# IONIQ6000/av1-go

Hardware: AMD Instinct MI355X
Metric: encoded 4K30 frames/sec (whole node) at fixed QP; PSNR-Y delta vs libaom (higher is better)
Workload: dtype u16

## Files before the change

### av1-go_amd/csrc/av1_entropy_kernels.hip

```cpp
#include <string.h>
#include <vector>
#include "av1_ops_cdfs.hpp"
#include "av1_ops32.hpp"
#include "av1mi_internal.hpp"

namespace av1mi {
using namespace av1ops;

struct Av1EntLaunch {
  FrameView fv;
  int nframes, sbr_n, sbc_n;
  BlockInfo *info;
  op_t *ops; uint32_t ops_cap;
  uint32_t *grouped; uint32_t grouped_cap;
  uint16_t *slot_total, *slot_base;
  uint16_t *rec;
  uint32_t *nops;
  uint8_t *slots; uint32_t slot_cap;
  uint32_t *tile_size;
  uint64_t *tile_off;
  uint32_t *status;
  uint8_t *out; uint64_t out_cap;
  const uint16_t *cdf_image; int cdf_words;
  SlotTable tab;
  const uint16_t *cdf_image32; SlotTable tab32;
  const uint8_t *lr_on_frame;
  int sb_rows32, band, nslots;
};

__device__ __forceinline__ FrameView frame_view(const Av1EntLaunch &L, int f) {
  FrameView v = L.fv;
  const long nb = (long)v.w8 * v.h8;
  if (v.key) { v.y_mode += nb * f; v.uv_mode += nb * f; }
  else { v.mv += nb * 2 * f; v.skip += nb * f; }
  v.lev_y += nb * 64 * f; v.lev_u += nb * 16 * f; v.lev_v += nb * 16 * f;
  v.info = L.info + nb * f;
  if (L.lr_on_frame) for (int p = 0; p < 3; p++) v.lr_on[p] = v.lr_on[p] && L.lr_on_frame[f * 3 + p];
  return v;
}

__global__ __launch_bounds__(256) void k_av1_info(Av1EntLaunch L) {
  const long nb = (long)L.fv.w8 * L.fv.h8, i = (long)blockIdx.x * 256 + threadIdx.x;
  if (i >= nb * L.nframes) return;
  const int f = (int)(i / nb), b = (int)(i - (long)f * nb);
  const FrameView v = frame_view(L, f);
  BlockInfo o = {};
  block_summary(v, b, &o);
  if (!v.key) inter_mode_decision(v, b / v.w8, b % v.w8, &o);
  L.info[nb * f + b] = o;
}

constexpr int kReplaySlots = (S_MAX + 1) / 2;
// ... 70 lines not shown
    if (sl >= S_MAX) continue;
    const bool on = sl < nslots;
    L.slot_total[(size_t)t * S_MAX + sl] = on ? S.total[sl] : (uint16_t)0;
    L.slot_base[(size_t)t * S_MAX + sl] = on ? S.base[sl] : (uint16_t)0;
  }
  op_t *list = L.ops + (size_t)t * L.ops_cap;
  uint32_t *grouped = L.grouped + (size_t)t * L.grouped_cap;
#pragma unroll
  for (int half = 0; half < 2; half++) {
    const int lo = half * kReplaySlots, hi = lo + kReplaySlots;
    if (half) __syncthreads();
#pragma unroll
    for (int q = 0; q < kOwn; q++) {
      const int sl = zi + 64 * q;
      if (sl < lo || sl >= hi || sl >= nslots) continue;
      int run = S.base[sl];
#pragma unroll
      for (int w = 0; w < kBlocksPerTile / 4; w++) {
        const uint32_t u = c[q][w];
        const int p0 = run, p1 = p0 + (int)(u & 0xFF), p2 = p1 + (int)((u >> 8) & 0xFF), p3 = p2 + (int)((u >> 16) & 0xFF);
        run = p3 + (int)(u >> 24);
        uint32_t *d = reinterpret_cast<uint32_t *>(S.pos + (sl - lo) * kBlocksPerTile + 4 * w);
        d[0] = (uint32_t)p0 | ((uint32_t)p1 << 16); d[1] = (uint32_t)p2 | ((uint32_t)p3 << 16);
      }
    }
    __syncthreads();
    __threadfence_block();
    replay_block(rec, k.nrec, S.pos, zi, first, list, grouped, lo, hi, half == 0);
  }
}

constexpr int kTiles32 = 16;
static_assert(kBlocks32 * kMag32Bytes >= K_END * kBlocks32 * 2 && kMag32Bytes % 8 == 0, "a tile's counters live where its four magnitude maps were");
__global__ __launch_bounds__(64) void k_av1_tokens32(Av1EntLaunch L, int ntiles_all) {
  __shared__ ScanTables32 scan;
  __shared__ __attribute__((aligned(16))) uint8_t s_mag[64 * kMag32Bytes];
  __shared__ Sum32 s_sum[kTiles32][kBlocks32];
  __shared__ int s_n[kTiles32][kBlocks32], s_nrec[kTiles32][kBlocks32], s_bad[kTiles32];
  const int tiles = L.sbr_n * L.sbc_n, tl = threadIdx.x >> 2, b = threadIdx.x & 3, t = blockIdx.x * kTiles32 + tl;
  bool live = t < ntiles_all;
  int f = 0, sbr = 0, sbc = 0;
  if (live) { f = t / tiles; const int tt = t - f * tiles; sbr = tt / L.sbc_n; sbc = tt - sbr * L.sbc_n; live = sbr < L.sb_rows32; }
  fill_scan_tables32(&scan, (int)threadIdx.x, 64);
  if (b == 0) s_bad[tl] = 0;
  const FrameView v = frame_view(L, live ? f : 0);
  const bool inside = live && !((b & 1) && sbc * 8 + 4 >= v.w8);
  if (inside) block_sums32(v, block_index32(v, sbr, sbc, b), &s_sum[tl][b]);
  __syncthreads();
  uint16_t *rec = L.rec + ((size_t)(live ? t : 0) * kBlocks32 + b) * kBlockRecords32;
  int nrec = 0;
  if (live) { s_n[tl][b] = 0; s_nrec[tl][b] = 0; }
  if (inside) {
    Sink32 k = { rec, nullptr, b, (int)kBlockRecords32, 0, 0, false, 0, 0, 0, 0 };
    const TokScratch32 ts = { s_mag + threadIdx.x * kMag32Bytes, &scan };
    tok_block32(v, k, ts, sbr, sbc, b, s_sum[tl]);
    s_n[tl][b] = k.n; s_nrec[tl][b] = nrec = k.nrec;
    if (k.overflow) atomicOr(&s_bad[tl], 1);
  }
  __syncthreads();
  uint16_t *cnt = reinterpret_cast<uint16_t *>(s_mag + tl * kBlocks32 * kMag32Bytes);
  for (int i = b; i < K_END * kBlocks32; i += kBlocks32) cnt[i] = 0;
  __syncthreads();
  if (live && !count_block32(rec, nrec, cnt, b)) atomicOr(&s_bad[tl], 1);
  __syncthreads();
  if (live && b == 0) {
    uint16_t *total = L.slot_total + (size_t)t * S_MAX, *base = L.slot_base + (size_t)t * S_MAX;
    const int run = place_tile32(cnt, total, base);
    for (int sl = K_END; sl < S_MAX; sl++) { total[sl] = 0; base[sl] = 0; }
    const int n = s_n[tl][0] + s_n[tl][1] + s_n[tl][2] + s_n[tl][3];
    if (s_bad[tl] || (uint32_t)n > L.ops_cap || run > 65535) {
      s_bad[tl] = 1;
      atomicOr(L.status, 1u);
      L.nops[t] = 0;
      for (int sl = 0; sl < K_END; sl++) total[sl] = 0;
    } else {
      L.nops[t] = (uint32_t)n;
    }
  }
  __syncthreads();
  if (!live || s_bad[tl]) return;
  int first = 0;
  for (int q = 0; q < b; q++) first += s_n[tl][q];
  replay_block32(rec, nrec, cnt, b, first, L.ops + (size_t)t * L.ops_cap, L.grouped + (size_t)t * L.grouped_cap);
}

__global__ __launch_bounds__(64) void k_av1_chains(Av1EntLaunch L, int ntiles_all, int ngroups) {
  const int xcd = blockIdx.x & 7, j = blockIdx.x >> 3, nslots = L.nslots;
  const int g = (j / nslots) * 8 + xcd, sl = j - (j / nslots) * nslots, lane = threadIdx.x, t = g * 64 + lane;
  if (g >= ngroups) return;
// ... 13 lines not shown
    const uint4 *g4 = reinterpret_cast<const uint4 *>(grouped);
    const uint4 z = make_uint4(0, 0, 0, 0);
    uint4 c0 = cnt > 0 ? g4[0] : z, c1 = cnt > 4 ? g4[1] : z, c2 = cnt > 8 ? g4[2] : z, c3 = cnt > 12 ? g4[3] : z;
    auto four = [&](const uint4 &v, int e) {
      if (e < cnt) list[v.x >> 4] = small_step(cdf, (int)(v.x & 15), n);
      if (e + 1 < cnt) list[v.y >> 4] = small_step(cdf, (int)(v.y & 15), n);
      if (e + 2 < cnt) list[v.z >> 4] = small_step(cdf, (int)(v.z & 15), n);
      if (e + 3 < cnt) list[v.w >> 4] = small_step(cdf, (int)(v.w & 15), n);
    };
#pragma unroll 1
    for (int e = 0; e < cnt; e += 16) {
      const uint4 *nx = g4 + (e >> 2) + 4;
      const uint4 n0 = e + 16 < cnt ? nx[0] : z, n1 = e + 20 < cnt ? nx[1] : z, n2 = e + 24 < cnt ? nx[2] : z, n3 = e + 28 < cnt ? nx[3] : z;
      four(c0, e); four(c1, e + 4); four(c2, e + 8); four(c3, e + 12);
      c0 = n0; c1 = n1; c2 = n2; c3 = n3;
    }
  } else {
    uint16_t *cdf = s_big + lane * 16;
    {
      const uint4 *iw = reinterpret_cast<const uint4 *>(L.cdf_image + off);
      uint4 *d = reinterpret_cast<uint4 *>(cdf);
      d[0] = iw[0];
      d[1] = n > 8 ? iw[1] : make_uint4(0, 0, 0, 0);
    }
#pragma unroll 1
    for (int e = 0; e < cnt; e++) {
      const uint32_t v = grouped[e];
      const int s = (int)(v & 15);
      list[v >> 4] = s >= kSplitHorz ? split_tuple(cdf, s) : big_step(cdf, s, n);
    }
  }
}

constexpr int kRingOps = 64, kLaneWords = kRingOps * 2 + Coder::kStage + 8;

__global__ __launch_bounds__(64) void k_av1_code(Av1EntLaunch L, int ntiles_all) {
  __shared__ __attribute__((aligned(16))) uint16_t s_lane[64 * kLaneWords];
  const int lane = threadIdx.x, t = blockIdx.x * 64 + lane;
  const bool live = t < ntiles_all;
  uint32_t *ring = reinterpret_cast<uint32_t *>(s_lane + lane * kLaneWords);
  Coder c;
  c.init(L.slots + (size_t)(live ? t : 0) * L.slot_cap, (int)L.slot_cap, s_lane + lane * kLaneWords + kRingOps * 2);
  const int n = live ? (int)L.nops[t] : 0;
  const uint4 *ops4 = reinterpret_cast<const uint4 *>(L.ops + (size_t)(live ? t : 0) * L.ops_cap);
  uint4 r0, r1, r2, r3, r4, r5, r6, r7;
  r0 = r1 = r2 = r3 = r4 = r5 = r6 = r7 = make_uint4(0, 0, 0, 0);
  int w = 0;
  bool pend = false;
  auto request = [&]() {
    const uint4 *p = ops4 + (w >> 2);
    if (w < n) r0 = p[0];
    if (w + 4 < n) r1 = p[1];
    if (w + 8 < n) r2 = p[2];
    if (w + 12 < n) r3 = p[3];
    if (w + 16 < n) r4 = p[4];
    if (w + 20 < n) r5 = p[5];
    if (w + 24 < n) r6 = p[6];
    if (w + 28 < n) r7 = p[7];
    pend = w < n;
  };
  auto take = [&]() {
    uint4 *q = reinterpret_cast<uint4 *>(ring + (w & 32));
    q[0] = r0; q[1] = r1; q[2] = r2; q[3] = r3; q[4] = r4; q[5] = r5; q[6] = r6; q[7] = r7;
    w += 32;
  };
  request();
  if (pend) { take(); request(); }
  int i = 0, lit_left = 0;
  uint32_t op = ring[0], op_next = ring[1], op_next2 = ring[2];
  for (;;) {
    if (!__any(lit_left > 0 || i < n)) break;
    if (__any((pend && w - i < 24) || c.ns >= Coder::kStage - 8)) {
      if (pend && w - i <= 32) { take(); request(); }
      c.spill();
    }
#pragma unroll
    for (int q = 0; q < 8; q++) {
      if (lit_left > 0 || i < n) {
        const uint32_t fetched = ring[(i + 3) & (kRingOps - 1)];
        uint32_t tup = op;
        if (lit_left == 0 && (op >> 31)) lit_left = (int)((op >> 27) & 15);
        if (lit_left > 0) {
          lit_left--;
          tup = (op >> lit_left) & 1 ? (1u << 19) | (256u << 9) : (2u << 19) | (512u << 9) | 256u;
        }
        c.encode_tuple(tup);
        if (lit_left == 0) { i++; op = op_next; op_next = op_next2; op_next2 = fetched; }
      }
    }
  }
  if (!live) return;
  int sz = n ? c.finish() : -1;
  if (sz < 0) { if (n) atomicOr(L.status, 2u); sz = 0; }
  L.tile_size[t] = (uint32_t)sz;
}

__global__ __launch_bounds__(1024) void k_av1_scan(Av1EntLaunch L, int ntiles_all) {
  __shared__ uint64_t part[1024];
  const int tid = threadIdx.x, per = (ntiles_all + 1023) / 1024, i0 = tid * per, i1 = min(i0 + per, ntiles_all);
  uint64_t s = 0;
  for (int i = i0; i < i1; i++) s += L.tile_size[i];
  part[tid] = s;
  __syncthreads();
  for (int d = 1; d < 1024; d <<= 1) {
    const uint64_t y = tid >= d ? part[tid - d] : 0;
    __syncthreads();
    part[tid] += y;
    __syncthreads();
  }
  uint64_t run = part[tid] - s;
  for (int i = i0; i < i1; i++) { L.tile_off[i] = run; run += L.tile_size[i]; }
  if (tid == 1023) {
    L.tile_off[ntiles_all] = part[1023];
    if (part[1023] > L.out_cap) atomicOr(L.status, 4u);
  }
}
__global__ __launch_bounds__(64) void k_av1_gather(Av1EntLaunch L) {
  const int t = blockIdx.x;
  const uint32_t n = L.tile_size[t];
  const uint64_t off = L.tile_off[t];
  if (off + n > L.out_cap) return;
  const uint8_t *src = L.slots + (size_t)t * L.slot_cap;
  uint8_t *dst = L.out + off;
  const uint32_t head = min(n, (uint32_t)((16 - (reinterpret_cast<uintptr_t>(dst) & 15)) & 15)), body = (n - head) >> 4, tail0 = head + (body << 4);
  if (threadIdx.x < head) dst[threadIdx.x] = src[threadIdx.x];
  for (uint32_t i = threadIdx.x; i < body; i += 64) {
    uint4 v;
    __builtin_memcpy(&v, src + head + 16 * i, 16);
    *reinterpret_cast<uint4 *>(dst + head + 16 * i) = v;
  }
  if (tail0 + threadIdx.x < n) dst[tail0 + threadIdx.x] = src[tail0 + threadIdx.x];
}

hipError_t launch_av1_front(av1mi_ctx *ctx, const Av1EntLaunch &L, hipStream_t s) {
  const long nb = (long)L.fv.w8 * L.fv.h8 * L.nframes;
  const int ntiles_all = L.sbr_n * L.sbc_n * L.nframes, ngroups = (ntiles_all + 63) / 64;
  ProfToken t = ctx_prof_begin(ctx, AV1MI_K_ENTROPY_TOKENS, s);
  hipLaunchKernelGGL(k_av1_info, dim3((unsigned)((nb + 255) / 256)), dim3(256), 0, s, L);
  if (L.sb_rows32 < L.sbr_n) hipLaunchKernelGGL(k_av1_tokens, dim3((unsigned)ntiles_all), dim3(64), 0, s, L);
  if (L.sb_rows32) hipLaunchKernelGGL(k_av1_tokens32, dim3((unsigned)((ntiles_all + kTiles32 - 1) / kTiles32)), dim3(64), 0, s, L, ntiles_all);
  ctx_prof_end(ctx, t, s);
  t = ctx_prof_begin(ctx, AV1MI_K_ENTROPY_CHAINS, s);
  Av1EntLaunch C = L;
  C.nslots = L.fv.key ? S_KEY_END : S_INTER_END; C.band = L.sb_rows32 ? 2 : 0;
  if (L.sb_rows32 < L.sbr_n) hipLaunchKernelGGL(k_av1_chains, dim3((unsigned)(((ngroups + 7) / 8) * 8 * C.nslots)), dim3(64), 0, s, C, ntiles_all, ngroups);
  if (L.sb_rows32) {
    C.nslots = K_END; C.band = 1; C.tab = L.tab32; C.cdf_image = L.cdf_image32;
    hipLaunchKernelGGL(k_av1_chains, dim3((unsigned)(((ngroups + 7) / 8) * 8 * C.nslots)), dim3(64), 0, s, C, ntiles_all, ngroups);
  }
  ctx_prof_end(ctx, t, s);
  return hipGetLastError();
}
hipError_t launch_av1_back(av1mi_ctx *ctx, const Av1EntLaunch &L, hipStream_t s) {
  const int ntiles_all = L.sbr_n * L.sbc_n * L.nframes;
  ProfToken t = ctx_prof_begin(ctx, AV1MI_K_ENTROPY, s);
  hipLaunchKernelGGL(k_av1_code, dim3((unsigned)((ntiles_all + 63) / 64)), dim3(64), 0, s, L, ntiles_all);
  ctx_prof_end(ctx, t, s);
  t = ctx_prof_begin(ctx, AV1MI_K_ENTROPY_PACK, s);
  hipLaunchKernelGGL(k_av1_scan, dim3(1), dim3(1024), 0, s, L, ntiles_all);
  hipLaunchKernelGGL(k_av1_gather, dim3((unsigned)ntiles_all), dim3(64), 0, s, L);
  ctx_prof_end(ctx, t, s);
  return hipGetLastError();
}

}

struct av1mi_av1ent_state {
  void *info = nullptr, *ops[2] = { nullptr, nullptr }, *nops[2] = { nullptr, nullptr }, *grouped = nullptr, *slot_tb = nullptr, *rec = nullptr, *slots = nullptr, *tile_off = nullptr, *status = nullptr;
  size_t info_b = 0, ops_b[2] = { 0, 0 }, nops_b[2] = { 0, 0 }, grouped_b = 0, slot_tb_b = 0, rec_b = 0, slots_b = 0, off_b = 0;
  hipEvent_t lists_ready[2] = { nullptr, nullptr }, lists_free[2] = { nullptr, nullptr };
  bool free_recorded[2] = { false, false };
  unsigned long jobs = 0;
  av1mi::Av1EntLaunch pending[2];
  uint64_t *pending_total[2] = { nullptr, nullptr };
  bool pending_valid[2] = { false, false };
  size_t last_tiles = 0;
  uint16_t *d_image[2][4] = {};
  uint16_t *d_image32[4] = {};
  av1ops::SlotTable tab32;
  int image_words[2] = { 0, 0 };
  av1ops::SlotTable tab[2];
};

namespace {
int grow(av1mi_ctx *ctx, void **p, size_t *have, size_t need) {
  if (*have >= need) return AV1MI_OK;
  if (*p) (void)hipFree(*p);
  *p = nullptr; *have = 0;
  if (hipMalloc(p, need) != hipSuccess) return av1mi::ctx_fail(ctx, AV1MI_E_NOMEM, "AV1 entropy scratch: hipMalloc(%zu) failed", need);
  *have = need;
  return AV1MI_OK;
}
}

extern "C" {

uint32_t av1mi_av1_entropy_ops_per_tile(void) { return 32768; }
uint32_t av1mi_av1_entropy_slot_bytes(void) { return 16384; }

}

int av1mi::av1_entropy_front(av1mi_ctx *ctx, const av1mi_av1_entropy_job *j, hipStream_t front, int *ticket) {
// ... 23 lines not shown
    return av1mi::ctx_fail(ctx, AV1MI_E_INVAL, "key_rows32 %d: whole superblock rows of a key frame whose width is a multiple of 32", j->key_rows32);
  if (j->key_rows32 && !st->d_image32[qcat]) {
    const std::vector<uint16_t> img = av1ops::default_slot_image_k32(qcat, &st->tab32);
    if (hipMalloc((void **)&st->d_image32[qcat], img.size() * 2) != hipSuccess ||
        hipMemcpy(st->d_image32[qcat], img.data(), img.size() * 2, hipMemcpyHostToDevice) != hipSuccess)
      return av1mi::ctx_fail(ctx, AV1MI_E_DEVICE, "uploading the default CDF image failed");
  }
  av1mi::Av1EntLaunch L;
  memset(&L, 0, sizeof(L));
  L.sb_rows32 = j->key_rows32 / 64;
  if (j->key_rows32) { av1ops::build_slot_table_k32(&L.tab32); L.cdf_image32 = st->d_image32[qcat]; }
  L.fv.w8 = j->width / 8; L.fv.h8 = j->height / 8; L.fv.key = key;
  L.fv.y_mode = j->d_modes_y; L.fv.uv_mode = j->d_modes_uv; L.fv.mv = j->d_mvs; L.fv.skip = j->d_skip;
  L.fv.lev_y = j->d_lev_y; L.fv.lev_u = j->d_lev_u; L.fv.lev_v = j->d_lev_v;
  for (int p = 0; p < 3; p++) {
    L.fv.lr_on[p] = j->lr_on[p] != 0;
    const int vh = j->visible_height ? j->visible_height : j->height, vw = j->visible_width ? j->visible_width : j->width;
    const int ph = p ? (vh + 1) / 2 : vh, pw = p ? (vw + 1) / 2 : vw;
    L.fv.lr_rows[p] = (ph + 32) / 64 > 1 ? (ph + 32) / 64 : 1; L.fv.lr_cols[p] = (pw + 32) / 64 > 1 ? (pw + 32) / 64 : 1;
  }
  memcpy(L.fv.lr_unit[0], j->lr_unit_y, 8); memcpy(L.fv.lr_unit[1], j->lr_unit_uv, 8);
  L.nframes = j->nframes; L.sbr_n = (L.fv.h8 + 7) / 8; L.sbc_n = (L.fv.w8 + 7) / 8;
  const size_t nb = (size_t)L.fv.w8 * L.fv.h8 * j->nframes, nt = (size_t)L.sbr_n * L.sbc_n * j->nframes;
  L.ops_cap = av1mi_av1_entropy_ops_per_tile(); L.slot_cap = av1mi_av1_entropy_slot_bytes();
  L.grouped_cap = L.ops_cap + av1ops::kListAlign * av1ops::S_MAX;
  const int par = (int)(st->jobs++ & 1);
  st->last_tiles = nt;
  int rc;
  if ((rc = grow(ctx, &st->info, &st->info_b, nb * sizeof(av1ops::BlockInfo))) ||
      (rc = grow(ctx, &st->ops[par], &st->ops_b[par], nt * L.ops_cap * sizeof(av1ops::op_t))) || (rc = grow(ctx, &st->nops[par], &st->nops_b[par], nt * 4)) ||
      (rc = grow(ctx, &st->grouped, &st->grouped_b, nt * L.grouped_cap * sizeof(uint32_t))) ||
      (rc = grow(ctx, &st->slot_tb, &st->slot_tb_b, nt * av1ops::S_MAX * 4)) ||
      (rc = grow(ctx, &st->rec, &st->rec_b, nt * av1ops::kBlocksPerTile * av1ops::kBlockRecords * sizeof(uint16_t))) ||
      (rc = grow(ctx, &st->slots, &st->slots_b, nt * L.slot_cap)) || (rc = grow(ctx, &st->tile_off, &st->off_b, (nt + 1) * 8)))
    return rc;
  L.info = (av1ops::BlockInfo *)st->info; L.ops = (av1ops::op_t *)st->ops[par]; L.nops = (uint32_t *)st->nops[par]; L.grouped = (uint32_t *)st->grouped;
  L.slot_total = (uint16_t *)st->slot_tb; L.slot_base = L.slot_total + nt * av1ops::S_MAX; L.rec = (uint16_t *)st->rec; L.slots = (uint8_t *)st->slots;
  L.tile_off = (uint64_t *)st->tile_off;
  L.tile_size = j->d_tile_size; L.out = j->d_out; L.out_cap = j->out_cap;
  L.status = (uint32_t *)(j->d_total + 1);
  L.cdf_image = st->d_image[key][qcat]; L.cdf_words = st->image_words[key]; L.tab = st->tab[key];
  L.lr_on_frame = j->d_lr_on;
#define E_HIP(call) do { const hipError_t e_ = (call); if (e_ != hipSuccess) return av1mi::ctx_fail(ctx, AV1MI_E_DEVICE, "%s: %s", #call, hipGetErrorString(e_)); } while (0)
  for (hipEvent_t *ev : { &st->lists_ready[par], &st->lists_free[par] }) if (!*ev) E_HIP(hipEventCreateWithFlags(ev, hipEventDisableTiming));
  if (st->free_recorded[par]) E_HIP(hipStreamWaitEvent(front, st->lists_free[par], 0));
  E_HIP(hipMemsetAsync(j->d_total, 0, 16, front));
  E_HIP(av1mi::launch_av1_front(ctx, L, front));
  E_HIP(hipEventRecord(st->lists_ready[par], front));
  st->pending[par] = L; st->pending_total[par] = j->d_total; st->pending_valid[par] = true;
  *ticket = par;
  return AV1MI_OK;
}

int av1mi::av1_entropy_back(av1mi_ctx *ctx, int ticket, hipStream_t back) {
  if (!ctx || ticket < 0 || ticket > 1) return AV1MI_E_INVAL;
  av1mi_av1ent_state *st = av1mi::ctx_av1ent(ctx);
  if (!st || !st->pending_valid[ticket]) return av1mi::ctx_fail(ctx, AV1MI_E_INVAL, "no entropy job pending under this ticket");
  const av1mi::Av1EntLaunch &L = st->pending[ticket];
  const size_t nt = (size_t)L.sbr_n * L.sbc_n * L.nframes;
  E_HIP(hipStreamWaitEvent(back, st->lists_ready[ticket], 0));
  E_HIP(av1mi::launch_av1_back(ctx, L, back));
  E_HIP(hipMemcpyAsync(st->pending_total[ticket], L.tile_off + nt, 8, hipMemcpyDeviceToDevice, back));
  E_HIP(hipEventRecord(st->lists_free[ticket], back)); st->free_recorded[ticket] = true;
  st->pending_valid[ticket] = false;
#undef E_HIP
  return AV1MI_OK;
}

int av1mi::av1_entropy_submit(av1mi_ctx *ctx, const av1mi_av1_entropy_job *j, hipStream_t front, hipStream_t back) {
  int ticket = -1;
  const int rc = av1_entropy_front(ctx, j, front, &ticket);
  if (rc != AV1MI_OK || ticket < 0) return rc;
  return av1_entropy_back(ctx, ticket, back);
}

extern "C" {

int av1mi_av1_entropy_encode_on(av1mi_ctx *ctx, const av1mi_av1_entropy_job *j, void *stream_handle) {
  if (!ctx) return AV1MI_E_INVAL;
  hipStream_t s = stream_handle ? (hipStream_t)stream_handle : av1mi::ctx_stream(ctx);
  return av1mi::av1_entropy_submit(ctx, j, s, s);
}

int av1mi_av1_entropy_encode(av1mi_ctx *ctx, const av1mi_av1_entropy_job *j) { return av1mi_av1_entropy_encode_on(ctx, j, nullptr); }

int av1mi_av1_entropy_last_list_words(av1mi_ctx *ctx, uint64_t *words) {
  if (!ctx || !words) return AV1MI_E_INVAL;
  *words = 0;
  av1mi_av1ent_state *st = av1mi::ctx_av1ent(ctx);
  if (!st || !st->jobs || !st->last_tiles) return AV1MI_OK;
  if (hipSetDevice(av1mi::ctx_device(ctx)) != hipSuccess || hipDeviceSynchronize() != hipSuccess) return av1mi::ctx_fail(ctx, AV1MI_E_DEVICE, "synchronising failed");
  std::vector<uint32_t> n(st->last_tiles);
  if (hipMemcpy(n.data(), st->nops[(st->jobs - 1) & 1], n.size() * 4, hipMemcpyDeviceToHost) != hipSuccess) return av1mi::ctx_fail(ctx, AV1MI_E_DEVICE, "reading the list sizes failed");
  for (uint32_t v : n) *words += v;
  return AV1MI_OK;
}

}

namespace av1mi {
void av1ent_free(av1mi_av1ent_state *st) {
  if (!st) return;
  for (void *p : { st->info, st->ops[0], st->ops[1], st->nops[0], st->nops[1], st->grouped, st->slot_tb, st->rec, st->slots, st->tile_off }) if (p) (void)hipFree(p);
  for (hipEvent_t ev : { st->lists_ready[0], st->lists_ready[1], st->lists_free[0], st->lists_free[1] }) if (ev) (void)hipEventDestroy(ev);
  for (auto &k : st->d_image) for (uint16_t *p : k) if (p) (void)hipFree(p);
  delete st;
}
av1mi_av1ent_state *av1ent_new() { return new (std::nothrow) av1mi_av1ent_state(); }
}
```

### av1-go_amd/csrc/av1_ops.hpp

```cpp
#pragma once
#include <stdint.h>

#if defined(__HIPCC__)
#include <hip/hip_runtime.h>
#define AV1_HD __host__ __device__ inline
#define AV1_UNROLL _Pragma("unroll")
#define AV1_NOUNROLL _Pragma("unroll 1")
#else
#define AV1_HD inline
#define AV1_UNROLL
#define AV1_NOUNROLL
#endif

namespace av1ops {

typedef uint32_t __attribute__((may_alias)) u32a;
typedef uint64_t __attribute__((may_alias)) u64a;

enum Slot : int {
  S_SKIP = 0,
  S_PART8 = S_SKIP + 3,
  S_PART16 = S_PART8 + 1,
  S_PART32 = S_PART16 + 4,
  S_PART64 = S_PART32 + 4,
// ... 591 lines not shown
    if (k >= nd) continue;
    uint32_t lo = adapt(w[k] & 0xFFFFu, 2 * k < s, rate), hi = adapt(w[k] >> 16, 2 * k + 1 < s, rate);
    if (k == nd - 1) hi = cnt + (cnt < 32);
    d[k] = lo | (hi << 16);
  }
  return make_tuple(fl, fh, s, n);
}

AV1_HD op_t split_tuple(const uint16_t *p, int kind) {
  const uint32_t p1 = p[0] - p[1], p2 = p[1] - p[2], p3 = p[2] - p[3], p4 = p[3] - p[4], p5 = p[4] - p[5], p6 = p[5] - p[6], p7 = p[6] - p[7],
                 p8 = p[7] - p[8], p9 = p[8];
  return make_tuple(kind == kSplitHorz ? p2 + p3 + p4 + p6 + p7 + p9 : p1 + p3 + p4 + p5 + p6 + p8, 0, 1, 2);
}

AV1_HD void run_chain(const uint16_t *init, int n, const uint32_t *g, int cnt, op_t *list) {
  if (n <= 4) {
    uint64_t w = (uint64_t)init[0] | ((uint64_t)init[1] << 16) | ((uint64_t)init[2] << 32) | ((uint64_t)init[3] << 48);
    for (int k = 0; k < cnt; k++) list[g[k] >> 4] = small_step(w, (int)(g[k] & 15), n);
    return;
  }
  alignas(16) uint16_t v[16];
  for (int i = 0; i < 16; i++) v[i] = i < slot_words(n) ? init[i] : 0;
  for (int k = 0; k < cnt; k++) {
    const int s = (int)(g[k] & 15);
    list[g[k] >> 4] = s >= kSplitHorz ? split_tuple(v, s) : big_step(v, s, n);
  }
}

AV1_HD void code_word(Coder &c, op_t e) {
  if (e >> 31) { for (int i = (int)((e >> 27) & 15) - 1; i >= 0; i--) { c.bit((e >> i) & 1); if (c.stage_full()) c.spill(); } }
  else { c.encode_tuple(e); if (c.stage_full()) c.spill(); }
}

}
```

### av1-go_amd/host/av1_opstream.cpp

```cpp
#include <algorithm>
#include <cstdio>
#include <cstdlib>
#include <cstring>
#include <string>
#include <vector>
#include "../csrc/av1_ops_cdfs.hpp"
#include "av1_bitstream.hpp"

namespace av1mi_host {
namespace av1 {

bool opstream_supported(const av1mi_obu_frame &f, std::string *why) {
  auto no = [&](const char *m) { if (why) *why = m; return false; };
  if (f.cdef_bits || f.reduced_tx_set || f.disable_cdf_update) return no("cdef_bits / reduced_tx_set / disable_cdf_update must be 0");
  if (f.tile_cols_log2 >= 0 || f.tile_rows_log2 >= 0) return no("one superblock per tile only");
  if (f.angle_y || f.angle_uv || f.cfl_alpha || f.tx_type || f.is_inter) return no("angle deltas, chroma from luma, transform types and intra blocks in inter frames are host-writer only");
  if (f.frame_type == 0 && f.skip) return no("key frames are coded with skip = 0");
  for (int p = 0; p < 3; p++) if (f.lr_type[p] > 1) return no("Wiener restoration only");
  if (f.lr_unit_shift || f.lr_uv_shift) return no("64x64 restoration units only");
  return true;
}

bool opstream_tiles(const av1mi_obu_frame &f, std::vector<std::vector<uint8_t>> *tiles, std::string *err, int key_rows32) {
  using namespace av1ops;
  if (!opstream_supported(f, err)) return false;
  if (key_rows32 && (f.frame_type != 0 || (key_rows32 & 63) || key_rows32 > f.height || (f.width & 31))) { if (err) *err = "bad 32x32 band"; return false; }
  FrameView v;
  memset(&v, 0, sizeof(v));
  v.w8 = f.width / 8; v.h8 = f.height / 8; v.key = f.frame_type == 0;
  v.y_mode = f.y_mode; v.uv_mode = f.uv_mode; v.mv = f.mv; v.skip = f.skip; v.lev_y = f.lev_y; v.lev_u = f.lev_u; v.lev_v = f.lev_v;
  std::vector<uint8_t> zskip;
  if (!v.key && !v.skip) { zskip.assign((size_t)v.w8 * v.h8, 0); v.skip = zskip.data(); }
  for (int p = 0; p < 3; p++) {
    v.lr_on[p] = f.lr_type[p] == 1;
    const int ph = p ? (visible_height(f) + 1) >> 1 : visible_height(f), pw = p ? (visible_width(f) + 1) >> 1 : visible_width(f);
    v.lr_rows[p] = std::max((ph + 32) / 64, 1); v.lr_cols[p] = std::max((pw + 32) / 64, 1);
  }
  for (int p = 0; p < 3; p++) {
    if (!v.lr_on[p]) continue;
    const int8_t *u = f.lr_units[p];
    const size_t n = (size_t)v.lr_rows[p] * v.lr_cols[p];
    for (size_t i = 1; i < n; i++) if (memcmp(u, u + i * 8, 8)) { if (err) *err = "restoration units must be uniform per plane"; return false; }
    if (p == 2 && v.lr_on[1] && memcmp(u, f.lr_units[1], 8)) { if (err) *err = "U and V restoration units must be equal"; return false; }
    memcpy(v.lr_unit[p ? 1 : 0], u, 8);
  }
  const size_t nb = (size_t)v.w8 * v.h8;
  std::vector<BlockInfo> info(nb);
  v.info = info.data();
  for (size_t b = 0; b < nb; b++) { memset(&info[b], 0, sizeof(BlockInfo)); block_summary(v, (int)b, &info[b]); }
  if (!v.key) for (int r = 0; r < v.h8; r++) for (int c = 0; c < v.w8; c++) inter_mode_decision(v, r, c, &info[(size_t)r * v.w8 + c]);
  const int qcat = f.base_q_idx <= 20 ? 0 : f.base_q_idx <= 60 ? 1 : f.base_q_idx <= 120 ? 2 : 3;
  SlotTable tab;
  const std::vector<uint16_t> image = default_slot_image(v.key != 0, qcat, &tab);
// ... 21 lines not shown
      if (sbr * 64 < key_rows32) {
        std::fill(cnt32.begin(), cnt32.end(), 0);
        const TokScratch32 ts32 = { mag32, scan32.data() };
        Sum32 sums[kBlocks32];
        const bool half = sbc * 8 + 4 >= v.w8;
        for (int b = 0; b < kBlocks32; b++) if (!(half && (b & 1))) block_sums32(v, block_index32(v, sbr, sbc, b), &sums[b]);
        int nrec[kBlocks32], first[kBlocks32 + 1];
        first[0] = 0;
        for (int b = 0; b < kBlocks32; b++) {
          Sink32 k = { &rec32[(size_t)b * kBlockRecords32], cnt32.data(), b, (int)kBlockRecords32, 0, 0, false, 0, 0, 0, 0 };
          tok_block32(v, k, ts32, sbr, sbc, b, sums);
          if (k.overflow) { if (err) *err = "a block exceeds the tokenizer's record area"; return false; }
          nrec[b] = k.nrec; first[b + 1] = first[b] + k.n;
        }
        for (int b = 0; b < kBlocks32; b++)
          if (!count_block32(&rec32[(size_t)b * kBlockRecords32], nrec[b], cnt32.data(), b)) { if (err) *err = "too many symbols of one slot in a block"; return false; }
        uint16_t base[K_END], total[K_END];
        const int run = place_tile32(cnt32.data(), total, base);
        if (run > 65535) { if (err) *err = "tile too large for 16-bit entry positions"; return false; }
        const int nops = first[kBlocks32];
        list.assign((size_t)nops, 0);
        grouped.assign((size_t)run, 0);
        for (int b = 0; b < kBlocks32; b++) replay_block32(&rec32[(size_t)b * kBlockRecords32], nrec[b], cnt32.data(), b, first[b], list.data(), grouped.data());
        for (int sl = 0; sl < K_END; sl++)
          if (total[sl]) run_chain(&image32[tab32.off[sl]], tab32.nsym[sl], &grouped[(size_t)base[sl]], total[sl], list.data());
        std::vector<uint8_t> &out = (*tiles)[(size_t)sbr * sbc_n + sbc];
        out.resize((size_t)nops * 2 + 64);
        Coder c;
        uint16_t stage[Coder::kStage];
        c.init(out.data(), (int)out.size(), stage);
        for (int i = 0; i < nops; i++) code_word(c, list[(size_t)i]);
        const int n = c.finish();
        if (n < 0) { if (err) *err = "tile payload overflow"; return false; }
        out.resize((size_t)n);
        continue;
      }
      std::fill(cnt.begin(), cnt.end(), 0);
      int first[kBlocksPerTile + 1], nrec[kBlocksPerTile];
      first[0] = 0;
      bool over = false;
      for (int zi = 0; zi < kBlocksPerTile; zi++) {
        Sink k = { &rec[(size_t)zi * kBlockRecords], cnt.data(), zi, 0, 0, false };
        tok_block(v, k, ts, sbr, sbc, zi);
        if (k.overflow && !stats) { if (err) *err = "a block exceeds the tokenizer's record area"; return false; }
        over |= k.overflow;
        nrec[zi] = k.nrec;
        first[zi + 1] = first[zi] + k.n;
        if (k.nrec > st_rec) st_rec = k.nrec;
      }
      if (stats) {
        for (uint8_t c : cnt) if (c > st_cnt) st_cnt = c;
        if (first[kBlocksPerTile] > st_ops) st_ops = first[kBlocksPerTile];
        st_ops_sum += first[kBlocksPerTile];
        if (over) { st_over++; continue; }
      }
      const int nops = first[kBlocksPerTile];
      int base[S_MAX], total[S_MAX], run = 0;
      for (int sl = 0; sl < nslots; sl++) {
        base[sl] = run;
        total[sl] = group_positions(&cnt[(size_t)sl * kBlocksPerTile], &pos[(size_t)sl * kBlocksPerTile], run);
        run = (run + total[sl] + kListAlign - 1) & ~(kListAlign - 1);
      }
      if (run > 65535) { if (err) *err = "tile too large for 16-bit entry positions"; return false; }
      list.assign((size_t)nops, 0);
      grouped.assign((size_t)run, 0);
      for (int zi = 0; zi < kBlocksPerTile; zi++)
        replay_block(&rec[(size_t)zi * kBlockRecords], nrec[zi], pos.data(), zi, first[zi], list.data(), grouped.data());
      for (int sl = 0; sl < nslots; sl++)
        if (total[sl]) run_chain(&image[tab.off[sl]], tab.nsym[sl], &grouped[(size_t)base[sl]], total[sl], list.data());
      std::vector<uint8_t> &out = (*tiles)[(size_t)sbr * sbc_n + sbc];
      out.resize((size_t)nops * 2 + 64);
      Coder c;
      uint16_t stage[Coder::kStage];
      c.init(out.data(), (int)out.size(), stage);
      for (int i = 0; i < nops; i++) code_word(c, list[(size_t)i]);
      const int n = c.finish();
      if (n < 0) { if (err) *err = "tile payload overflow"; return false; }
      out.resize((size_t)n);
    }
  if (stats)
    fprintf(stderr, "[av1mi tok stats] %d tiles: records per block <= %d (capacity %d), symbols of a slot in a block <= %d (255), list words per tile <= %d, mean %.0f; %d tiles over a block capacity\n",
            sbr_n * sbc_n, st_rec, (int)kBlockRecords, st_cnt, st_ops, (double)st_ops_sum / (sbr_n * sbc_n), st_over);
  return true;
}

}
}
```

### av1-go_amd/host/coder_selftest.cpp

```cpp
#include <stdint.h>
#include <string.h>
#include <vector>
#include "av1_bitstream.hpp"
#define AV1_CODER_STATS
namespace coder_selftest {
#include "../csrc/av1_ops.hpp"
}

extern "C" long long av1mi_host_coder_selftest(uint64_t seed, long long count, long long *carries) {
  using coder_selftest::av1ops::Coder;
  std::vector<uint32_t> fl((size_t)count), fh((size_t)count);
  std::vector<uint8_t> sy((size_t)count), ns((size_t)count);
  uint64_t x = seed * 0x9E3779B97F4A7C15ull + 1;
  auto rnd = [&]() { x ^= x << 13; x ^= x >> 7; x ^= x << 17; return (uint32_t)(x >> 16); };
  for (long long i = 0; i < count; i++) {
    const int n = 2 + (int)(rnd() % 15);
    int s;
    uint32_t a, b;
    s = (int)(rnd() % (uint32_t)n);
    const uint32_t hi = 32768u - 64u * (uint32_t)s, lo = 64u * (uint32_t)(n - 1 - s);
    a = s == 0 ? 32768u : lo + 64u + rnd() % (hi - lo - 63u);
    b = s == n - 1 ? 0u : lo + rnd() % (a - 63u - lo);
    fl[(size_t)i] = a; fh[(size_t)i] = b; sy[(size_t)i] = (uint8_t)s; ns[(size_t)i] = (uint8_t)n;
  }
  const std::vector<uint8_t> ref = av1mi_host::av1::range_code_raw(fl.data(), fh.data(), sy.data(), ns.data(), (size_t)count);
  std::vector<uint8_t> out((size_t)count * 2 + 64);
  coder_selftest::av1ops::coder_stat_carries = 0;
  Coder c;
  uint16_t stage[Coder::kStage];
  c.init(out.data(), (int)out.size(), stage);
  for (long long i = 0; i < count; i++) {
    c.encode(fl[(size_t)i], fh[(size_t)i], sy[(size_t)i], ns[(size_t)i]);
    if (c.stage_full()) c.spill();
  }
  const int sz = c.finish();
  if (carries) *carries = coder_selftest::av1ops::coder_stat_carries;
  if (sz < 0 || (size_t)sz != ref.size()) return -1;
  for (size_t i = 0; i < ref.size(); i++) if (out[i] != ref[i]) return (long long)i + 1;
  return 0;
}
```

Measured before the change: 2807.

## Split range coding into cut-point pass plus parallel chunked bit emission

The per-tile range coder, which ran one tile per lane serially, is split into two kernels. A first pass tracks only the range and bit count and logs cut points. A second kernel then encodes up to 64 chunks of each tile in parallel, one per lane, and resolves cross-chunk carries with a wavefront generate/propagate scan. This aims to turn the serial entropy-coding bottleneck into wide parallel work. The cost is a second pass over the op list, an extra launch, a new cuts buffer, and intricate carry logic that is checked by new host self-tests.

```diff
diff --git a/av1-go_amd/csrc/av1_entropy_kernels.hip b/av1-go_amd/csrc/av1_entropy_kernels.hip
--- a/av1-go_amd/csrc/av1_entropy_kernels.hip
+++ b/av1-go_amd/csrc/av1_entropy_kernels.hip
@@ -18,6 +18,7 @@
   uint32_t *nops;
   uint8_t *slots; uint32_t slot_cap;
   uint32_t *tile_size;
+  uint2 *cuts;
   uint64_t *tile_off;
   uint32_t *status;
   uint8_t *out; uint64_t out_cap;
@@ -154,6 +155,7 @@
 
 constexpr int kTiles32 = 16;
 static_assert(kBlocks32 * kMag32Bytes >= K_END * kBlocks32 * 2 && kMag32Bytes % 8 == 0, "a tile's counters live where its four magnitude maps were");
+static_assert(kBlockRecords32 >= 10 * (1024 + 2 * 256) + 1024, "a 32x32 block's worst-case records fit its record area");
 __global__ __launch_bounds__(64) void k_av1_tokens32(Av1EntLaunch L, int ntiles_all) {
   __shared__ ScanTables32 scan;
   __shared__ __attribute__((aligned(16))) uint8_t s_mag[64 * kMag32Bytes];
@@ -176,7 +178,7 @@
     Sink32 k = { rec, nullptr, b, (int)kBlockRecords32, 0, 0, false, 0, 0, 0, 0 };
     const TokScratch32 ts = { s_mag + threadIdx.x * kMag32Bytes, &scan };
     tok_block32(v, k, ts, sbr, sbc, b, s_sum[tl]);
-    s_n[tl][b] = k.n; s_nrec[tl][b] = nrec = k.nrec;
+    s_n[tl][b] = k.n; s_nrec[tl][b] = nrec = k.overflow ? imin(k.nrec, (int)kBlockRecords32) & ~7 : k.nrec;
     if (k.overflow) atomicOr(&s_bad[tl], 1);
   }
   __syncthreads();
@@ -256,22 +258,14 @@
   }
 }
 
-constexpr int kRingOps = 64, kLaneWords = kRingOps * 2 + Coder::kStage + 8;
-
-__global__ __launch_bounds__(64) void k_av1_code(Av1EntLaunch L, int ntiles_all) {
-  __shared__ __attribute__((aligned(16))) uint16_t s_lane[64 * kLaneWords];
-  const int lane = threadIdx.x, t = blockIdx.x * 64 + lane;
-  const bool live = t < ntiles_all;
-  uint32_t *ring = reinterpret_cast<uint32_t *>(s_lane + lane * kLaneWords);
-  Coder c;
-  c.init(L.slots + (size_t)(live ? t : 0) * L.slot_cap, (int)L.slot_cap, s_lane + lane * kLaneWords + kRingOps * 2);
-  const int n = live ? (int)L.nops[t] : 0;
-  const uint4 *ops4 = reinterpret_cast<const uint4 *>(L.ops + (size_t)(live ? t : 0) * L.ops_cap);
+constexpr int kRingOps = 64, kRingWords = kRingOps + 4;
+struct ListRing {
+  const uint4 *ops4;
+  uint32_t *ring;
+  int n, w;
+  bool pend;
   uint4 r0, r1, r2, r3, r4, r5, r6, r7;
-  r0 = r1 = r2 = r3 = r4 = r5 = r6 = r7 = make_uint4(0, 0, 0, 0);
-  int w = 0;
-  bool pend = false;
-  auto request = [&]() {
+  __device__ void request() {
     const uint4 *p = ops4 + (w >> 2);
     if (w < n) r0 = p[0];
     if (w + 4 < n) r1 = p[1];
@@ -282,41 +276,128 @@
     if (w + 24 < n) r6 = p[6];
     if (w + 28 < n) r7 = p[7];
     pend = w < n;
-  };
-  auto take = [&]() {
+  }
+  __device__ void take() {
     uint4 *q = reinterpret_cast<uint4 *>(ring + (w & 32));
     q[0] = r0; q[1] = r1; q[2] = r2; q[3] = r3; q[4] = r4; q[5] = r5; q[6] = r6; q[7] = r7;
     w += 32;
-  };
-  request();
-  if (pend) { take(); request(); }
-  int i = 0, lit_left = 0;
+  }
+  __device__ void start(const op_t *ops, uint32_t *rg, int nwords, int from) {
+    ops4 = reinterpret_cast<const uint4 *>(ops); ring = rg; n = nwords; w = from & ~31;
+    r0 = r1 = r2 = r3 = r4 = r5 = r6 = r7 = make_uint4(0, 0, 0, 0);
+    request();
+    if (pend) { take(); request(); }
+    if (pend) { take(); request(); }
+  }
+  __device__ void phase(int i) {
+    if (__any(pend && w - i < 24)) { if (pend && w - i <= 32) { take(); request(); } }
+  }
+};
+
+__global__ __launch_bounds__(64) void k_av1_code(Av1EntLaunch L, int ntiles_all) {
+  __shared__ __attribute__((aligned(16))) uint32_t s_ring[64 * kRingWords];
+  __shared__ uint32_t s_cut[2][(kCodeCuts - 1) * 64];
+  const int lane = threadIdx.x, t = blockIdx.x * 64 + lane;
+  const bool live = t < ntiles_all;
+  const int n = live ? (int)L.nops[t] : 0;
+  ListRing R;
+  R.start(L.ops + (size_t)(live ? t : 0) * L.ops_cap, s_ring + lane * kRingWords, n, 0);
+  const uint32_t *ring = R.ring;
+  CutLog cuts;
+  cuts.init(s_cut[0] + lane, s_cut[1] + lane, 64, kCutBits);
+  uint32_t rng = 0x8000;
+  int S = 0, i = 0, lit_left = 0;
   uint32_t op = ring[0], op_next = ring[1], op_next2 = ring[2];
   for (;;) {
     if (!__any(lit_left > 0 || i < n)) break;
-    if (__any((pend && w - i < 24) || c.ns >= Coder::kStage - 8)) {
-      if (pend && w - i <= 32) { take(); request(); }
-      c.spill();
-    }
+    R.phase(i);
+    if (lit_left == 0 && i < n && S >= cuts.thr) cuts.cut(i, rng, S);
 #pragma unroll
     for (int q = 0; q < 8; q++) {
-      if (lit_left > 0 || i < n) {
-        const uint32_t fetched = ring[(i + 3) & (kRingOps - 1)];
-        uint32_t tup = op;
-        if (lit_left == 0 && (op >> 31)) lit_left = (int)((op >> 27) & 15);
-        if (lit_left > 0) {
-          lit_left--;
-          tup = (op >> lit_left) & 1 ? (1u << 19) | (256u << 9) : (2u << 19) | (512u << 9) | 256u;
-        }
-        c.encode_tuple(tup);
-        if (lit_left == 0) { i++; op = op_next; op_next = op_next2; op_next2 = fetched; }
-      }
+      const uint32_t fetched = ring[(i + 3) & (kRingOps - 1)];
+      const bool on = lit_left > 0 || i < n;
+      const int nl = lit_left == 0 && (op >> 31) ? (int)((op >> 27) & 15) : lit_left;
+      const int ll = nl > 0 ? nl - 1 : 0;
+      const op_t tup = nl > 0 ? lit_tuple((op >> ll) & 1) : op;
+      uint32_t r = rng;
+      const int d = rng_step(r, tup);
+      rng = on ? r : rng;
+      S += on ? d : 0;
+      const bool adv = on && ll == 0;
+      lit_left = on ? ll : lit_left;
+      i += adv;
+      op = adv ? op_next : op; op_next = adv ? op_next2 : op_next; op_next2 = adv ? fetched : op_next2;
     }
   }
   if (!live) return;
-  int sz = n ? c.finish() : -1;
-  if (sz < 0) { if (n) atomicOr(L.status, 2u); sz = 0; }
-  L.tile_size[t] = (uint32_t)sz;
+  uint32_t sz = 0;
+  if (n) {
+    const int nc = cuts.finish(S);
+    uint2 *cp = L.cuts + (size_t)t * kCodeCuts;
+    cp[0] = make_uint2((uint32_t)nc, (uint32_t)S);
+    for (int j = 1; j < nc; j++) cp[j] = make_uint2(s_cut[0][(j - 1) * 64 + lane], s_cut[1][(j - 1) * 64 + lane]);
+    sz = (uint32_t)(S + 8) >> 3;
+    if (sz > L.slot_cap) { atomicOr(L.status, 2u); sz = 0; }
+  }
+  L.tile_size[t] = sz;
+}
+
+__global__ __launch_bounds__(64) void k_av1_code_bits(Av1EntLaunch L) {
+  __shared__ __attribute__((aligned(16))) uint32_t s_ring[64 * kRingWords];
+  const int t = blockIdx.x, k = threadIdx.x;
+  const uint32_t size = L.tile_size[t];
+  if (!size) return;
+  const uint2 *cp = L.cuts + (size_t)t * kCodeCuts;
+  const uint2 h = cp[0];
+  const int nc = (int)h.x;
+  const bool live = k < nc, last = k == nc - 1;
+  const uint2 a = live && k ? cp[k] : make_uint2(0x8000u << 16, 0u);
+  const uint2 b = k + 1 < nc ? cp[k + 1] : make_uint2(L.nops[t], h.y);
+  const int i0 = live ? (int)(a.x & 0xFFFFu) : 0, i1 = live ? (int)(b.x & 0xFFFFu) : 0;
+  ChunkCoder c;
+  c.init(L.slots + (size_t)t * L.slot_cap, (int)size, k, a.x >> 16, (int)a.y);
+  ListRing R;
+  R.start(L.ops + (size_t)t * L.ops_cap, s_ring + k * kRingWords, i1, i0);
+  const uint32_t *ring = R.ring;
+  int i = i0, lit_left = 0;
+  uint32_t op = ring[i & (kRingOps - 1)], op_next = ring[(i + 1) & (kRingOps - 1)], op_next2 = ring[(i + 2) & (kRingOps - 1)];
+  for (;;) {
+    if (!__any(lit_left > 0 || i < i1)) break;
+    R.phase(i);
+#pragma unroll
+    for (int q = 0; q < 8; q++) {
+      const uint32_t fetched = ring[(i + 3) & (kRingOps - 1)];
+      const bool on = lit_left > 0 || i < i1;
+      const int nl = lit_left == 0 && (op >> 31) ? (int)((op >> 27) & 15) : lit_left;
+      const int ll = nl > 0 ? nl - 1 : 0;
+      const op_t tup = nl > 0 ? lit_tuple((op >> ll) & 1) : op;
+      if (on) c.encode_tuple(tup);
+      const bool adv = on && ll == 0;
+      lit_left = on ? ll : lit_left;
+      i += adv;
+      op = adv ? op_next : op; op_next = adv ? op_next2 : op_next; op_next2 = adv ? fetched : op_next2;
+    }
+  }
+  uint32_t lo = 0;
+  if (live) { if (last) c.end_last(); else lo = c.end_mid((int)b.y); }
+  const uint32_t hn = __shfl_down(c.hi, 1, 64);
+  int g = 0, p = 0;
+  if (live && !last) {
+    const uint64_t s = (uint64_t)lo + hn;
+    lo = (uint32_t)s;
+    if (s >> 32) g = c.carry_back();
+    p = !c.top && lo == 0xFFFFFFFFu && c.middle_all_ones();
+  }
+#pragma unroll
+  for (int d = 1; d < 64; d <<= 1) {
+    const int g2 = __shfl_down(g, d, 64), p2 = __shfl_down(p, d, 64);
+    if (k + d < 64) { g |= p & g2; p &= p2; }
+  }
+  const int cin = __shfl_down(g, 1, 64);
+  if (live && !last) {
+    if (cin && ++lo == 0) c.carry_back();
+    c.put_lo(lo);
+  }
 }
 
 __global__ __launch_bounds__(1024) void k_av1_scan(Av1EntLaunch L, int ntiles_all) {
@@ -379,6 +460,7 @@
   const int ntiles_all = L.sbr_n * L.sbc_n * L.nframes;
   ProfToken t = ctx_prof_begin(ctx, AV1MI_K_ENTROPY, s);
   hipLaunchKernelGGL(k_av1_code, dim3((unsigned)((ntiles_all + 63) / 64)), dim3(64), 0, s, L, ntiles_all);
+  hipLaunchKernelGGL(k_av1_code_bits, dim3((unsigned)ntiles_all), dim3(64), 0, s, L);
   ctx_prof_end(ctx, t, s);
   t = ctx_prof_begin(ctx, AV1MI_K_ENTROPY_PACK, s);
   hipLaunchKernelGGL(k_av1_scan, dim3(1), dim3(1024), 0, s, L, ntiles_all);
@@ -392,6 +474,8 @@
 struct av1mi_av1ent_state {
   void *info = nullptr, *ops[2] = { nullptr, nullptr }, *nops[2] = { nullptr, nullptr }, *grouped = nullptr, *slot_tb = nullptr, *rec = nullptr, *slots = nullptr, *tile_off = nullptr, *status = nullptr;
   size_t info_b = 0, ops_b[2] = { 0, 0 }, nops_b[2] = { 0, 0 }, grouped_b = 0, slot_tb_b = 0, rec_b = 0, slots_b = 0, off_b = 0;
+  void *cuts = nullptr;
+  size_t cuts_b = 0;
   hipEvent_t lists_ready[2] = { nullptr, nullptr }, lists_free[2] = { nullptr, nullptr };
   bool free_recorded[2] = { false, false };
   unsigned long jobs = 0;
@@ -481,11 +565,12 @@
       (rc = grow(ctx, &st->grouped, &st->grouped_b, nt * L.grouped_cap * sizeof(uint32_t))) ||
       (rc = grow(ctx, &st->slot_tb, &st->slot_tb_b, nt * av1ops::S_MAX * 4)) ||
       (rc = grow(ctx, &st->rec, &st->rec_b, nt * av1ops::kBlocksPerTile * av1ops::kBlockRecords * sizeof(uint16_t))) ||
-      (rc = grow(ctx, &st->slots, &st->slots_b, nt * L.slot_cap)) || (rc = grow(ctx, &st->tile_off, &st->off_b, (nt + 1) * 8)))
+      (rc = grow(ctx, &st->slots, &st->slots_b, nt * L.slot_cap)) || (rc = grow(ctx, &st->tile_off, &st->off_b, (nt + 1) * 8)) ||
+      (rc = grow(ctx, &st->cuts, &st->cuts_b, nt * av1ops::kCodeCuts * sizeof(uint2))))
     return rc;
   L.info = (av1ops::BlockInfo *)st->info; L.ops = (av1ops::op_t *)st->ops[par]; L.nops = (uint32_t *)st->nops[par]; L.grouped = (uint32_t *)st->grouped;
   L.slot_total = (uint16_t *)st->slot_tb; L.slot_base = L.slot_total + nt * av1ops::S_MAX; L.rec = (uint16_t *)st->rec; L.slots = (uint8_t *)st->slots;
-  L.tile_off = (uint64_t *)st->tile_off;
+  L.tile_off = (uint64_t *)st->tile_off; L.cuts = (uint2 *)st->cuts;
   L.tile_size = j->d_tile_size; L.out = j->d_out; L.out_cap = j->out_cap;
   L.status = (uint32_t *)(j->d_total + 1);
   L.cdf_image = st->d_image[key][qcat]; L.cdf_words = st->image_words[key]; L.tab = st->tab[key];
@@ -550,7 +635,7 @@
 namespace av1mi {
 void av1ent_free(av1mi_av1ent_state *st) {
   if (!st) return;
-  for (void *p : { st->info, st->ops[0], st->ops[1], st->nops[0], st->nops[1], st->grouped, st->slot_tb, st->rec, st->slots, st->tile_off }) if (p) (void)hipFree(p);
+  for (void *p : { st->info, st->ops[0], st->ops[1], st->nops[0], st->nops[1], st->grouped, st->slot_tb, st->rec, st->slots, st->tile_off, st->cuts }) if (p) (void)hipFree(p);
   for (hipEvent_t ev : { st->lists_ready[0], st->lists_ready[1], st->lists_free[0], st->lists_free[1] }) if (ev) (void)hipEventDestroy(ev);
   for (auto &k : st->d_image) for (uint16_t *p : k) if (p) (void)hipFree(p);
   delete st;
diff --git a/av1-go_amd/csrc/av1_ops.hpp b/av1-go_amd/csrc/av1_ops.hpp
--- a/av1-go_amd/csrc/av1_ops.hpp
+++ b/av1-go_amd/csrc/av1_ops.hpp
@@ -647,4 +647,177 @@
   else { c.encode_tuple(e); if (c.stage_full()) c.spill(); }
 }
 
-}
+constexpr int kCodeCuts = 64;
+constexpr int kCutBits = 64;
+constexpr int kChunkMinBits = 48;
+
+AV1_HD op_t lit_tuple(unsigned b) { return b ? (1u << 19) | (256u << 9) : (2u << 19) | (512u << 9) | 256u; }
+
+AV1_HD int rng_step(uint32_t &rng, op_t t) {
+  const uint32_t fl6 = (t >> 9) & 1023u, fh6 = t & 511u, dl = (t >> 19) & 31u;
+  const uint32_t r = rng, v = (((r >> 8) * fh6) >> 1) + 4u * (dl - 1u);
+  const uint32_t u = fl6 < 512u ? (((r >> 8) * fl6) >> 1) + 4u * dl : r;
+  const uint32_t nr = u - v;
+  const int d = 15 - ilog2(nr);
+  rng = nr << d;
+  return d;
+}
+
+#ifdef AV1_CODER_STATS
+static long long coder_stat_compactions = 0, coder_stat_rounding_carries = 0, coder_stat_overhang_carries = 0, coder_stat_generates = 0,
+                 coder_stat_crossings = 0, coder_stat_propagates = 0;
+#endif
+struct CutLog {
+  uint32_t *iw, *sh;
+  int stride, cnt, bits, thr;
+  AV1_HD void init(uint32_t *a, uint32_t *b, int s, int bits0) { iw = a; sh = b; stride = s; cnt = 0; bits = bits0; thr = bits0; }
+  AV1_HD void cut(int i, uint32_t rng, int S) {
+    if (cnt == kCodeCuts - 1) {
+#ifdef AV1_CODER_STATS
+      coder_stat_compactions++;
+#endif
+      for (int j = 1; j < kCodeCuts / 2; j++) { iw[(j - 1) * stride] = iw[(2 * j - 1) * stride]; sh[(j - 1) * stride] = sh[(2 * j - 1) * stride]; }
+      cnt = kCodeCuts / 2 - 1;
+      bits *= 2;
+    }
+    iw[cnt * stride] = (uint32_t)i | (rng << 16);
+    sh[cnt * stride] = (uint32_t)S;
+    cnt++;
+    thr = S + bits;
+  }
+  AV1_HD int finish(int D) {
+    if (cnt && D - (int)sh[(cnt - 1) * stride] < kChunkMinBits) cnt--;
+    return cnt + 1;
+  }
+};
+
+struct ChunkCoder {
+  uint64_t low;
+  uint32_t rng, hi;
+  int nb, nhi, pos, lim;
+  uint8_t *out;
+  bool top;
+  AV1_HD void init(uint8_t *slot, int size, int k, uint32_t rng0, int S0) {
+    low = 0; rng = rng0; hi = 0; pos = 0;
+    top = k == 0;
+    if (top) { nb = -1; nhi = 2; out = slot; lim = size; return; }
+    const int a = (S0 - 1) >> 4;
+    nb = (S0 - 1) & 15; nhi = 0; out = slot + 2 * (a + 2); lim = size - 2 * (a + 2);
+  }
+  AV1_HD void store16(int p, uint32_t w) {
+    if (p + 2 <= lim) *reinterpret_cast<uint16_t *>(out + p) = (uint16_t)((w >> 8) | (w << 8));
+    else if (p < lim) out[p] = (uint8_t)(w >> 8);
+  }
+  AV1_HD void put(uint32_t w) {
+    if (nhi < 2) { hi = (hi << 16) | w; nhi++; return; }
+    store16(pos, w);
+    pos += 2;
+  }
+  AV1_HD bool carry_back() {
+    for (int i = pos < lim ? pos : lim; i-- > 0;) if (++out[i] != 0) return false;
+    if (top) return false;
+    hi++;
+    return true;
+  }
+  AV1_HD void flush16() {
+    nb -= 16;
+    const uint32_t w = (uint32_t)(low >> (16 + nb));
+    if (w >> 16) carry_back();
+    put(w & 0xFFFFu);
+    low &= ((uint64_t)1 << (16 + nb)) - 1;
+  }
+  AV1_HD void encode_tuple(op_t t) {
+    const uint32_t fl6 = (t >> 9) & 1023u, fh6 = t & 511u, dl = (t >> 19) & 31u;
+    const uint32_t r = rng, v = (((r >> 8) * fh6) >> 1) + 4u * (dl - 1u);
+    const uint32_t u = fl6 < 512u ? (((r >> 8) * fl6) >> 1) + 4u * dl : r;
+    low += r - u;
+    const uint32_t nr = u - v;
+    const int d = 15 - ilog2(nr);
+    rng = nr << d; low <<= d; nb += d;
+    if (nb >= 32) flush16();
+  }
+  AV1_HD uint32_t end_mid(int S1) {
+    if (low >> (16 + nb)) { carry_back(); low &= ((uint64_t)1 << (16 + nb)) - 1; }
+    const int pad = 16 - ((S1 - 1) & 15);
+    const uint64_t p = low << pad;
+    if (16 + nb + pad > 32) put((uint32_t)(p >> 32) & 0xFFFFu);
+    return (uint32_t)p;
+  }
+  AV1_HD void end_last() {
+    uint64_t e = ((low + 0x3FFF) & ~(uint64_t)0x3FFF) | 0x4000;
+    if (nb >= 0 && (e >> (16 + nb))) {
+#ifdef AV1_CODER_STATS
+      if (!(low >> (16 + nb))) coder_stat_rounding_carries++;
+#endif
+      carry_back();
+    }
+    const int bits = 16 + nb, pad = (16 - (bits & 15)) & 15;
+    e = (e & (((uint64_t)1 << bits) - 1)) << pad;
+    for (int q = (bits + pad) / 16 - 1; q >= 0; q--) put((uint32_t)(e >> (16 * q)) & 0xFFFFu);
+  }
+  AV1_HD bool middle_all_ones() const {
+    for (int i = 0; i < pos && i < lim; i++) if (out[i] != 0xFF) return false;
+    return true;
+  }
+  AV1_HD void put_lo(uint32_t lo) { store16(pos, lo >> 16); store16(pos + 2, lo & 0xFFFFu); }
+};
+
+AV1_HD void chunk_word(ChunkCoder &c, op_t e) {
+  if (e >> 31) { for (int b = (int)((e >> 27) & 15) - 1; b >= 0; b--) c.encode_tuple(lit_tuple((e >> b) & 1)); }
+  else c.encode_tuple(e);
+}
+
+inline int split_code(const op_t *list, int n, uint8_t *slot, int cap, uint32_t *iw, uint32_t *sh, int bits0 = kCutBits, int every = 1) {
+  if (n <= 0) return -1;
+  CutLog cuts;
+  cuts.init(iw, sh, 1, bits0);
+  uint32_t rng = 0x8000;
+  int D = 0;
+  for (int i = 0; i < n; i++) {
+    if (i % every == 0 && D >= cuts.thr) cuts.cut(i, rng, D);
+    const op_t e = list[i];
+    if (e >> 31) { for (int b = (int)((e >> 27) & 15) - 1; b >= 0; b--) D += rng_step(rng, lit_tuple((e >> b) & 1)); }
+    else D += rng_step(rng, e);
+  }
+  const int nc = cuts.finish(D), size = (D + 8) >> 3;
+  if (size > cap) return -1;
+  ChunkCoder c[kCodeCuts];
+  uint32_t lo[kCodeCuts], hi0[kCodeCuts];
+  bool g[kCodeCuts], p[kCodeCuts];
+  for (int k = 0; k < nc; k++) {
+    const int i0 = k ? (int)(iw[k - 1] & 0xFFFFu) : 0, i1 = k + 1 < nc ? (int)(iw[k] & 0xFFFFu) : n;
+    c[k].init(slot, size, k, k ? iw[k - 1] >> 16 : 0x8000u, k ? (int)sh[k - 1] : 0);
+    for (int i = i0; i < i1; i++) chunk_word(c[k], list[i]);
+    lo[k] = 0;
+    if (k + 1 < nc) lo[k] = c[k].end_mid((int)sh[k]);
+    else c[k].end_last();
+    hi0[k] = c[k].hi;
+  }
+  for (int k = 0; k < nc; k++) {
+    g[k] = p[k] = false;
+    if (k + 1 == nc) continue;
+    const uint64_t s = (uint64_t)lo[k] + hi0[k + 1];
+    lo[k] = (uint32_t)s;
+    if (s >> 32) g[k] = c[k].carry_back();
+    p[k] = !c[k].top && lo[k] == 0xFFFFFFFFu && c[k].middle_all_ones();
+#ifdef AV1_CODER_STATS
+    coder_stat_overhang_carries += (int)(s >> 32);
+    coder_stat_generates += g[k];
+#endif
+  }
+  bool cin = false;
+  for (int k = nc - 1; k >= 0; k--) {
+    if (k + 1 < nc) {
+#ifdef AV1_CODER_STATS
+      coder_stat_crossings += cin;
+      coder_stat_propagates += cin && p[k];
+#endif
+      if (cin && ++lo[k] == 0) c[k].carry_back();
+      c[k].put_lo(lo[k]);
+    }
+    cin = g[k] || (p[k] && cin);
+  }
+  return size;
+}
+
+}
diff --git a/av1-go_amd/host/av1_opstream.cpp b/av1-go_amd/host/av1_opstream.cpp
--- a/av1-go_amd/host/av1_opstream.cpp
+++ b/av1-go_amd/host/av1_opstream.cpp
@@ -19,6 +19,19 @@
   for (int p = 0; p < 3; p++) if (f.lr_type[p] > 1) return no("Wiener restoration only");
   if (f.lr_unit_shift || f.lr_uv_shift) return no("64x64 restoration units only");
   return true;
+}
+
+static bool g_split_check = false;
+static long long g_split_tiles = 0, g_split_bad = 0;
+static void split_check(const av1ops::op_t *list, int nops, const uint8_t *ref, int n) {
+  if (!g_split_check || nops <= 0) return;
+  uint32_t iw[av1ops::kCodeCuts], sh[av1ops::kCodeCuts];
+  for (int every : { 1, 8 }) {
+    std::vector<uint8_t> s((size_t)n + 16, 0xA5);
+    const int m = av1ops::split_code(list, nops, s.data(), n, iw, sh, av1ops::kCutBits, every);
+    g_split_tiles++;
+    if (m != n || memcmp(s.data(), ref, (size_t)n) || s[(size_t)n] != 0xA5) g_split_bad++;
+  }
 }
 
 bool opstream_tiles(const av1mi_obu_frame &f, std::vector<std::vector<uint8_t>> *tiles, std::string *err, int key_rows32) {
@@ -106,6 +119,7 @@
         for (int i = 0; i < nops; i++) code_word(c, list[(size_t)i]);
         const int n = c.finish();
         if (n < 0) { if (err) *err = "tile payload overflow"; return false; }
+        split_check(list.data(), nops, out.data(), n);
         out.resize((size_t)n);
         continue;
       }
@@ -150,6 +164,7 @@
       for (int i = 0; i < nops; i++) code_word(c, list[(size_t)i]);
       const int n = c.finish();
       if (n < 0) { if (err) *err = "tile payload overflow"; return false; }
+      split_check(list.data(), nops, out.data(), n);
       out.resize((size_t)n);
     }
   if (stats)
@@ -160,3 +175,11 @@
 
 }
 }
+
+extern "C" void av1mi_host_split_check(int on, long long *tiles, long long *bad) {
+  using namespace av1mi_host::av1;
+  if (tiles) *tiles = g_split_tiles;
+  if (bad) *bad = g_split_bad;
+  g_split_check = on != 0;
+  g_split_tiles = g_split_bad = 0;
+}
diff --git a/av1-go_amd/host/coder_selftest.cpp b/av1-go_amd/host/coder_selftest.cpp
--- a/av1-go_amd/host/coder_selftest.cpp
+++ b/av1-go_amd/host/coder_selftest.cpp
@@ -39,3 +39,55 @@
   for (size_t i = 0; i < ref.size(); i++) if (out[i] != ref[i]) return (long long)i + 1;
   return 0;
 }
+
+extern "C" long long av1mi_host_split_coder_selftest(uint64_t seed, long long lists, int mode, int bits0, int every, long long *stats) {
+  namespace A = coder_selftest::av1ops;
+  uint64_t x = seed * 0x9E3779B97F4A7C15ull + 7;
+  auto rnd = [&]() { x ^= x << 13; x ^= x >> 7; x ^= x << 17; return (uint32_t)(x >> 16); };
+  auto tuple = [&](bool probable) {
+    const int n = 2 + (int)(rnd() % 15), s = probable ? 0 : (int)(rnd() % (uint32_t)n);
+    const uint32_t hi = 32768u - 64u * (uint32_t)s, lo = 64u * (uint32_t)(n - 1 - s);
+    const uint32_t a = s == 0 ? 32768u : lo + 64u + rnd() % (hi - lo - 63u);
+    const uint32_t b = s == n - 1 ? 0u : probable ? lo + rnd() % 64u : lo + rnd() % (a - 63u - lo);
+    return A::make_tuple(a, b, s, n);
+  };
+  A::coder_stat_carries = A::coder_stat_compactions = A::coder_stat_rounding_carries = A::coder_stat_overhang_carries = 0;
+  A::coder_stat_generates = A::coder_stat_crossings = A::coder_stat_propagates = 0;
+  std::vector<A::op_t> list;
+  std::vector<uint8_t> ref, got;
+  uint32_t iw[A::kCodeCuts], sh[A::kCodeCuts];
+  uint16_t stage[A::Coder::kStage];
+  const int lit_pct = mode == 2 ? 80 : mode == 1 ? 2 : 20;
+  for (long long l = 0; l < lists; l++) {
+    const int len = mode == 3 ? (int)(rnd() % 9) : 1 + (int)(rnd() % 4000);
+    list.resize((size_t)len);
+    for (A::op_t &e : list) {
+      if ((int)(rnd() % 100) < lit_pct) e = A::op_lit(1 + (int)(rnd() % 11), mode == 2 && rnd() % 4 == 0 ? 0x7FFu : rnd());
+      else e = tuple(mode == 1 ? rnd() % 100 < 95 : rnd() % 100 < 30);
+    }
+    if (len == 0) {
+      if (A::split_code(list.data(), 0, nullptr, 0, iw, sh, bits0, every) != -1) return l + 1;
+      continue;
+    }
+    ref.assign((size_t)len * 24 + 64, 0);
+    A::Coder c;
+    c.init(ref.data(), (int)ref.size(), stage);
+    for (A::op_t e : list) A::code_word(c, e);
+    const int size = c.finish();
+    if (size <= 0) return l + 1;
+    std::vector<uint8_t> small((size_t)size);
+    c.init(small.data(), size - 1, stage);
+    for (A::op_t e : list) A::code_word(c, e);
+    if (c.finish() != -1) return l + 1;
+    got.assign((size_t)size + 16, 0xA5);
+    if (A::split_code(list.data(), len, got.data(), size, iw, sh, bits0, every) != size || memcmp(got.data(), ref.data(), (size_t)size)) return l + 1;
+    for (int i = size; i < size + 16; i++) if (got[(size_t)i] != 0xA5) return l + 1;
+    if (A::split_code(list.data(), len, got.data(), size - 1, iw, sh, bits0, every) != -1) return l + 1;
+  }
+  if (stats) {
+    const long long s[7] = { A::coder_stat_compactions, A::coder_stat_rounding_carries, A::coder_stat_overhang_carries, A::coder_stat_generates,
+                             A::coder_stat_crossings, A::coder_stat_propagates, A::coder_stat_carries };
+    memcpy(stats, s, sizeof(s));
+  }
+  return 0;
+}
```

Measured after the change: 2596, median of 2. 0.925x the previous value.
